# luoao-kddi/SCP

Hardware: AMD Instinct MI355X
Metric: KITTI frames/sec encode (SCP-EHEM, level 16) + bpp match vs ref (higher is better)
Workload: dtype f32 (dense layers and attention as bf16x3 split on bf16 MFMA, feature kNN as f16x3 split on f16 MFMA, fp32 accumulate; position kNN / CDF in fp32); 1 GPU; SCP-EHEM KITTI-like synthetic 120k-pt frames, --spher --mullevel lidar_level=16 (BASELINE.json configs[2]), seeded random weights; nodes_per_frame=577403, windows_per_frame=100, frames_per_gpu=46, frames_in_flight=4, frames_per_launch_sequence=1, transform=host-numpy on a prefetch thread (strict identity: the reference's integers), parallelism=frame-sharded x1, rank_cores=256, rank_cores_pinned=False

## Files before the change

### scp_amd/csrc/cdf.hip

```cpp
#include "scp_internal.h"

#define ROWS 64
#define MAXSYM 255

template <bool FROM_LOGITS>
__global__ __launch_bounds__(256) void cdf_kernel(const float *__restrict__ in, int64_t ld, int64_t n, int nsym,
                                                  const uint8_t *__restrict__ sym, float *__restrict__ pmf_out,
                                                  uint32_t *__restrict__ lohi, uint16_t *__restrict__ cdf_full) {
    __shared__ float tile[ROWS * MAXSYM];
    __shared__ float part[4 * ROWS];
    const int tid = threadIdx.x, lane = tid & 63, wq = tid >> 6;
    const int64_t row0 = (int64_t)blockIdx.x * ROWS;
    const int nrow = (int)((n - row0) < ROWS ? (n - row0) : ROWS);
    const int total = nrow * nsym;
    if (ld == nsym) {
        const float *src = in + row0 * ld;
        for (int i = tid; i < total; i += 256) tile[i] = src[i];
    } else if (ld == 256 && nsym <= 256 && (((uintptr_t)in) & 15) == 0) {
        for (int r = wq; r < nrow; r += 4) {
            const float4 v = *(const float4 *)(in + (row0 + r) * 256 + 4 * lane);
            const int c = 4 * lane;
            float *d = tile + r * nsym + c;
            if (c < nsym) d[0] = v.x;
            if (c + 1 < nsym) d[1] = v.y;
            if (c + 2 < nsym) d[2] = v.z;
            if (c + 3 < nsym) d[3] = v.w;
        }
    } else {
        for (int i = tid; i < total; i += 256) { const int r = i / nsym, c = i - r * nsym; tile[i] = in[(row0 + r) * ld + c]; }
    }
    __syncthreads();
    float *row = tile + lane * nsym;
// ... 41 lines not shown
            for (int u = 0; u < 8; ++u) v[u] = row[j + u];
#pragma unroll
            for (int u = 0; u < 8; ++u) { c = __fadd_rn(c, v[u]); v[u] = c; }
#pragma unroll
            for (int u = 0; u < 8; ++u) row[j + u] = v[u];
        }
        for (; j < nsym; ++j) { c = __fadd_rn(c, row[j]); row[j] = c; }
        const float c_last = c;
        const float c_lo = s > 0 ? row[s - 1] : 0.f, c_hi = row[s < nsym ? s : nsym - 1];
        if (lohi) {
            const double scale = (double)(65536 - nsym);
            const uint32_t lo = (s == 0) ? 0u : ((uint32_t)(int64_t)rint((double)(float)((double)c_lo / (double)c_last) * scale) + (uint32_t)s) & 0xFFFFu;
            uint32_t hi = ((uint32_t)(int64_t)rint((double)(float)((double)c_hi / (double)c_last) * scale) + (uint32_t)(s + 1)) & 0xFFFFu;
            if (s == nsym - 1) hi = 0u;
            lohi[row0 + lane] = lo | (hi << 16);
        }
    }
    if (cdf_full) {
        __syncthreads();
        const double scale = (double)(65536 - nsym);
        const int Lp = nsym + 1;
        for (int i = tid; i < nrow * Lp; i += 256) {
            const int r = i / Lp, k = i - r * Lp;
            uint32_t v = 0;
            if (k > 0) {
                const float last = tile[r * nsym + nsym - 1];
                v = ((uint32_t)(int64_t)rint((double)(float)((double)tile[r * nsym + k - 1] / (double)last) * scale) + (uint32_t)k) & 0xFFFFu;
            }
            cdf_full[(row0 + r) * Lp + k] = (uint16_t)v;
        }
    }
}

static int launch(bool from_logits, const float *in, int64_t ld, int64_t n, int32_t nsym, const uint8_t *sym, float *pmf,
                  uint32_t *lohi, uint16_t *cdf_full, void *stream) {
    if (n == 0) return SCP_OK;
    if (!in || n < 0 || nsym < 2 || nsym > MAXSYM || ld < nsym) return SCP_EINVAL;
    if (lohi && !sym) return SCP_EINVAL;
    const int nb = (int)cdiv64(n, ROWS);
    hipStream_t st = (hipStream_t)stream;
    SCP_PROF(SCP_PROF_CDF, st, (double)n * (4.0 * nsym + 4.0));
    if (from_logits) hipLaunchKernelGGL(cdf_kernel<true>, dim3(nb), dim3(256), 0, st, in, ld, n, nsym, sym, pmf, lohi, cdf_full);
    else hipLaunchKernelGGL(cdf_kernel<false>, dim3(nb), dim3(256), 0, st, in, ld, n, nsym, sym, pmf, lohi, cdf_full);
    LAUNCH_CHECK();
    return SCP_OK;
}

extern "C" int scp_softmax_cdf(const float *logits, int64_t ld, int64_t n, int32_t nsym, const uint8_t *sym, float *pmf,
                               uint32_t *lohi, uint16_t *cdf_full, void *stream) {
    return launch(true, logits, ld, n, nsym, sym, pmf, lohi, cdf_full, stream);
}

extern "C" int scp_pmf_cdf(const float *pmf, int64_t n, int32_t nsym, const uint8_t *sym, uint32_t *lohi, uint16_t *cdf_full,
                           void *stream) {
    return launch(false, pmf, nsym, n, nsym, sym, nullptr, lohi, cdf_full, stream);
}
```

### scp_amd/csrc/lnlin2.hip

```cpp
#include <stdlib.h>
#include <type_traits>
#include "rc_common.h"

#define L2_Q 16384
#define L2_OFF_BOUNCE (3 * L2_Q)
#define L2_OFF_BIAS (L2_OFF_BOUNCE + 4 * RC_BOUNCE)
#define L2_LDS (L2_OFF_BIAS + 8192)
static_assert(L2_LDS <= 80 * 1024, "two workgroups per CU: at most half of the 160 KiB");
#define L2_LDS_ONE (160 * 1024)

__device__ __forceinline__ void l2_issue(const RcLane &L, __amdgpu_buffer_rsrc_t wr_hi, __amdgpu_buffer_rsrc_t wr_lo, int j, int qt, char *dst) {
#pragma unroll
    for (int i = 0; i < 4; ++i) {
        const int b = i >> 1, plane = i & 1;
        const int soff = ((2 * j + b) * 16 + (L.w >> 1) * 8 + qt * 2 + (L.w & 1)) * 1024;
        __builtin_amdgcn_raw_ptr_buffer_load_lds(plane ? wr_lo : wr_hi, (rc_lds_ptr_t)(dst + (L.w + 4 * i) * 1024), 16, L.lane * 16, soff, 0, 0);
    }
}

#define L2_READ4(d0, d1, d2, d3, addr, o0, o1, o2, o3)                                                                                  \
    asm volatile("ds_read_b128 %0, %4 offset:%5\n\tds_read_b128 %1, %4 offset:%6\n\tds_read_b128 %2, %4 offset:%7\n\t"                      \
                 "ds_read_b128 %3, %4 offset:%8\n\ts_waitcnt lgkmcnt(0)"                                                                  \
                 : "=&v"(d0), "=&v"(d1), "=&v"(d2), "=&v"(d3) : "v"(addr), "n"(o0), "n"(o1), "n"(o2), "n"(o3) : "memory")
#define L2_READ4_AHEAD(d0, d1, d2, d3, addr, o0, o1, o2, o3)                                                                            \
    asm volatile("ds_read_b128 %0, %4 offset:%5\n\tds_read_b128 %1, %4 offset:%6\n\tds_read_b128 %2, %4 offset:%7\n\t"                      \
                 "ds_read_b128 %3, %4 offset:%8"                                                                                         \
                 : "=&v"(d0), "=&v"(d1), "=&v"(d2), "=&v"(d3) : "v"(addr), "n"(o0), "n"(o1), "n"(o2), "n"(o3) : "memory")
#define L2_WAIT4(d0, d1, d2, d3) asm volatile("s_waitcnt lgkmcnt(0)" : "+v"(d0), "+v"(d1), "+v"(d2), "+v"(d3) :: "memory")
#define L2_TOP(N) asm volatile("s_waitcnt vmcnt(" #N ") lgkmcnt(0)\n\ts_barrier" ::: "memory")

template <bool SWAP, int Q>
__device__ __forceinline__ void l2_quarter(unsigned ad0, unsigned ad1, rf32x16 &c0, rf32x16 &c1, const rbf16x8 (&Xh)[16], const rbf16x8 (&Xl)[16]) {
#define L2_MFMA(c, wf, xf) c = SWAP ? __builtin_amdgcn_mfma_f32_32x32x16_bf16(xf, wf, c, 0, 0, 0) : __builtin_amdgcn_mfma_f32_32x32x16_bf16(wf, xf, c, 0, 0, 0)
#define L2_FRAGS(M, A, ad, s) M(A[1], A[3], A[0], A[2], ad, 4096 + ((s) >> 1) * 1024, 12288 + ((s) >> 1) * 1024, ((s) >> 1) * 1024, 8192 + ((s) >> 1) * 1024)
    rbf16x8 A[2][4];
    L2_FRAGS(L2_READ4, A[0], ad0, 0);
#pragma unroll
    for (int s = 0; s < 4; ++s) {
        const int k = 4 * Q + s, n = (s + 1) & 1;
        if (s < 3) {
// ... 68 lines not shown
#pragma unroll
    for (int plane = 0; plane < 2; ++plane)
#pragma unroll
        for (int it = 0; it < 4; ++it)
            __builtin_amdgcn_raw_buffer_store_b128(y[plane][it], prs, L.lane * 16, it * 1024 + (vblk + head) * 4096 + (2 + plane) * pbytes, 0);
    asm volatile("s_waitcnt lgkmcnt(0)" ::: "memory");
}

template <bool KV>
__global__ __launch_bounds__(256, 2) void ln2_proj_kernel(const RcLnLinArgs a) {
    extern __shared__ __attribute__((aligned(1024))) char smem[];
    const RcLane L = rc_lane();
    const int ntiles = (a.M + RC_ROWS - 1) / RC_ROWS;
    const int nsteps = a.N >> 6;
    const int nq = KV ? a.nq : nsteps;
    char *bounce = smem + L2_OFF_BOUNCE + L.w * RC_BOUNCE;
    const unsigned ab = (unsigned)(uintptr_t)(rc_lds_ptr_t)smem + L.rg * 2048;
    const unsigned af0 = ab + L.frag, af1 = ab + (L.frag ^ 32);
    const unsigned asb = (unsigned)(uintptr_t)(rc_lds_ptr_t)(smem + L2_OFF_BIAS);
    const int ldo_bytes = (int)(a.ldo * 4);
    const int voff = (32 * L.w + (L.lane >> 3)) * ldo_bytes + (L.lane & 7) * 16;
    const int pbytes = (int)a.plane_bytes;
    const __amdgpu_buffer_rsrc_t prs = __builtin_amdgcn_make_buffer_rsrc((void *)a.planes, 0, (KV && !(a.probe & 1)) ? (int)(4 * a.plane_bytes) : 0, 0x00020000);
    const bool dma = !(a.probe & 2);

    const int wbytes = ((a.N + 255) & ~255) * 512;
    const __amdgpu_buffer_rsrc_t wr_hi = __builtin_amdgcn_make_buffer_rsrc((void *)a.Whi, 0, wbytes, 0x00020000);
    const __amdgpu_buffer_rsrc_t wr_lo = __builtin_amdgcn_make_buffer_rsrc((void *)a.Wlo, 0, wbytes, 0x00020000);

    float *sb = (float *)(smem + L2_OFF_BIAS), *sbw = sb + 1024;
    for (int i = threadIdx.x; i < a.N; i += 256) {
        const float b = a.bias ? a.bias[i] : 0.f;
        sb[i] = b; sbw[i] = b + (a.wbeta ? a.wbeta[i] : 0.f);
    }
    __syncthreads();
    int slot = 0;
    if (dma) { l2_issue(L, wr_hi, wr_lo, 0, 0, smem); l2_issue(L, wr_hi, wr_lo, 0, 1, smem + L2_Q); }
    for (int tile = blockIdx.x; tile < ntiles; tile += (int)gridDim.x) {
        const int m0 = tile * RC_ROWS;
        const int row = m0 + 32 * L.w + L.col;
        const int rowc = row < a.M ? row : a.M - 1;
        float keep = (row < a.M) ? 1.0f : 0.0f;
        if (a.valid) keep *= a.valid[rowc];
        rbf16x8 Xh[16], Xl[16];
        {
            float v[128];
            const float *src = a.x + (int64_t)((a.probe & 4) ? (rowc & 127) % a.M : rowc) * a.ldx + 8 * L.h;
#pragma unroll
            for (int s = 0; s < 16; ++s) {
                const rf32x4 q0 = *(const rf32x4 *)(src + 16 * s), q1 = *(const rf32x4 *)(src + 16 * s + 4);
#pragma unroll
                for (int u = 0; u < 4; ++u) { v[8 * s + u] = q0[u]; v[8 * s + 4 + u] = q1[u]; }
            }
            float mean, rstd;
            rc_ln_stats(v, a.eps, mean, rstd);
            const float sc = rstd * keep;
#pragma unroll
            for (int s = 0; s < 16; ++s) {
                float f[8];
#pragma unroll
                for (int i = 0; i < 8; ++i) f[i] = (v[8 * s + i] - mean) * sc;
                rc_split8(f, Xh[s], Xl[s]);
            }
        }
        const bool kept = keep != 0.f;
        const int64_t rows_left = (int64_t)a.M - m0;
        const int64_t span = (rows_left < RC_ROWS ? rows_left : RC_ROWS) * a.ldo * 4;
        const __amdgpu_buffer_rsrc_t rs = __builtin_amdgcn_make_buffer_rsrc(a.out + (int64_t)m0 * a.ldo, 0, (a.probe & 1) ? 0 : (int)span, 0x00020000);
        const unsigned kmask = (unsigned)__builtin_amdgcn_ballot_w64(kept);
        const unsigned maskh = kmask >> (4 * L.h);
        const int kvoff = (m0 + 32 * L.w + (L.lane >> 3)) * 512 + (L.lane & 7) * 16;
        const int vblk = ((m0 >> 5) + L.w) * 4;

        const unsigned atb = asb + (kept ? 4096 : 0) + 16 * L.h, atv = asb + 4 * L.col;
        rf32x16 c0, c1;
        auto bias_start = [&](int j) {
            if (KV && j >= nq + 4) {
                float bb[2], bwv[2];
                const unsigned ad = atv + 256 * j;
                asm volatile("ds_read_b32 %0, %4\n\tds_read_b32 %1, %4 offset:128\n\tds_read_b32 %2, %4 offset:4096\n\tds_read_b32 %3, %4 offset:4224\n\t"
                             "s_waitcnt lgkmcnt(0)" : "=&v"(bb[0]), "=&v"(bb[1]), "=&v"(bwv[0]), "=&v"(bwv[1]) : "v"(ad) : "memory");
#pragma unroll
                for (int blk = 0; blk < 2; ++blk) {
                    rf32x16 &c = blk ? c1 : c0;
#pragma unroll
                    for (int r = 0; r < 16; ++r) c[r] = ((maskh >> (8 * (r >> 2) + (r & 3))) & 1u) ? bwv[blk] : bb[blk];
                }
            } else {
                const unsigned ad = atb + 256 * j;
                rf32x4 t[2][4];
                L2_READ4(t[0][0], t[0][1], t[0][2], t[0][3], ad, 0, 32, 64, 96);
                L2_READ4(t[1][0], t[1][1], t[1][2], t[1][3], ad, 128, 160, 192, 224);
#pragma unroll
                for (int q = 0; q < 4; ++q)
#pragma unroll
                    for (int u = 0; u < 4; ++u) { c0[4 * q + u] = t[0][q][u]; c1[4 * q + u] = t[1][q][u]; }
            }
        };
        bias_start(0);
        SCP_WAIT_DMA(0);
        auto steps = [&](auto sw, int ja, int jb) {
// ... 16 lines not shown
            L2_QUARTER(3, 4)
#undef L2_QUARTER
            __builtin_amdgcn_sched_barrier(0);
            if (!SW && j < nq) {
#pragma unroll
                for (int blk = 0; blk < 2; ++blk) {
                    rf32x4 o[4];
#pragma unroll
                    for (int q = 0; q < 4; ++q)
#pragma unroll
                        for (int u = 0; u < 4; ++u) o[q][u] = (blk ? c1 : c0)[4 * q + u];
                    rc_store_block(L, bounce, o, rs, ldo_bytes, voff, 64 * j + 32 * blk);
                }
            } else if (!SW) {
                l2_store_k(L, bounce, c0, c1, prs, kvoff, pbytes, j - nq);
            } else {
                l2_store_v(L, bounce, c0, c1, prs, vblk, pbytes, j - nq - 4);
            }
            if (j + 1 < nsteps) bias_start(jn);
        }
        };
        if (KV) { steps(std::false_type(), 0, nq + 4); steps(std::true_type(), nq + 4, nsteps); }
        else steps(std::false_type(), 0, nsteps);
    }
    SCP_WAIT_DMA(0);
}

int scp_lnlin2_mode() {
    static int mode = -1;
    if (mode < 0) { const char *e = getenv("SCP_LNLIN"); mode = e ? atoi(e) : 0; if (mode < 0 || mode > 2) mode = 0; }
    return mode;
}

int scp_lnlin2_launch(RcLnLinArgs a, bool kv, int ncu, hipStream_t stream) {
    static int one = -1, probe = -1;
    if (one < 0) { const char *e = getenv("SCP_LNLIN_ONE"); one = (e && e[0] == '1') ? 1 : 0; }
    if (probe < 0) { const char *e = getenv("SCP_RC_PROBE"); probe = e ? atoi(e) : 0; }
    static bool configured = false;
    if (!configured) {
        HIP_TRY(hipFuncSetAttribute((const void *)ln2_proj_kernel<false>, hipFuncAttributeMaxDynamicSharedMemorySize, one ? L2_LDS_ONE : L2_LDS));
        HIP_TRY(hipFuncSetAttribute((const void *)ln2_proj_kernel<true>, hipFuncAttributeMaxDynamicSharedMemorySize, one ? L2_LDS_ONE : L2_LDS));
        configured = true;
    }
    a.ngroups = 1; a.probe = probe; a.dbg = nullptr;
    const int ntiles = (a.M + RC_ROWS - 1) / RC_ROWS;
    const int wgs = (one ? 1 : 2) * ncu;
    const dim3 grid((unsigned)(ntiles < wgs ? ntiles : wgs));
    if (kv) hipLaunchKernelGGL(ln2_proj_kernel<true>, grid, dim3(256), one ? L2_LDS_ONE : L2_LDS, stream, a);
    else hipLaunchKernelGGL(ln2_proj_kernel<false>, grid, dim3(256), one ? L2_LDS_ONE : L2_LDS, stream, a);
    LAUNCH_CHECK();
    return SCP_OK;
}
```

### scp_amd/csrc/rc_common.h

```cpp
#pragma once
#include "scp_internal.h"

typedef __bf16 rbf16x8 __attribute__((ext_vector_type(8)));
typedef float rf32x16 __attribute__((ext_vector_type(16)));
typedef float rf32x4 __attribute__((ext_vector_type(4)));
typedef int ri32x4 __attribute__((ext_vector_type(4)));
typedef __attribute__((address_space(3))) void *rc_lds_ptr_t;
typedef const __attribute__((address_space(1))) void *rc_glb_ptr_t;

#define RC_ROWS 128
#define RC_BOUNCE 4096

__device__ __forceinline__ void rc_dma16(const void *g, char *l) {
    __builtin_amdgcn_global_load_lds((rc_glb_ptr_t)g, (rc_lds_ptr_t)l, 16, 0, 0);
}

typedef float rf32x2 __attribute__((ext_vector_type(2)));
typedef __bf16 rbf16x2 __attribute__((ext_vector_type(2)));
typedef unsigned ru32x4 __attribute__((ext_vector_type(4)));
typedef unsigned ru32x2 __attribute__((ext_vector_type(2)));
__device__ __forceinline__ unsigned rc_pack2(float a, float b) {
    const rf32x2 v = {a, b};
    return __builtin_bit_cast(unsigned, __builtin_convertvector(v, rbf16x2));
}
// ... 38 lines not shown
        const int rho = 8 * it + (L.lane >> 3), kap = L.lane & 7;
        y[it] = *(const rf32x4 *)(bounce + rho * 128 + ((kap ^ (rho & 7)) << 4));
    }
#pragma unroll
    for (int it = 0; it < 4; ++it) __builtin_amdgcn_raw_buffer_store_b128(__builtin_bit_cast(ri32x4, y[it]), rs, voff, it * 8 * ldo_bytes + ch0 * 4, 0);
    asm volatile("s_waitcnt lgkmcnt(0)" ::: "memory");
}

__device__ __forceinline__ void rc_ln_stats(const float *v , float eps, float &mean, float &rstd) {
    float s = 0.f;
#pragma unroll
    for (int i = 0; i < 128; i += 4) s += (v[i] + v[i + 1]) + (v[i + 2] + v[i + 3]);
    s += __shfl_xor(s, 32);
    mean = s * (1.0f / 256.0f);
    float q = 0.f;
#pragma unroll
    for (int i = 0; i < 128; ++i) { const float d = v[i] - mean; q += d * d; }
    q += __shfl_xor(q, 32);
    rstd = rsqrtf(q * (1.0f / 256.0f) + eps);
}

struct RcLnLinArgs {
    const float *x; int64_t ldx;
    const float *valid;
    const __bf16 *Whi, *Wlo;
    const float *bias, *wbeta;
    float *out; int64_t ldo;
    int M, N;
    float eps;
    int probe;
    unsigned long long *dbg;
    __bf16 *planes; int64_t plane_bytes; int nq;
    int ngroups;
};

int scp_lnlin2_mode();
int scp_lnlin2_launch(RcLnLinArgs a, bool kv, int ncu, hipStream_t stream);
```

### scp_amd/csrc/rowchain.hip

```cpp
#include <stdlib.h>
#include "scp_internal.h"
#include "rc_common.h"

#define RC_SLOT 32768
#define RC_RING (4 * RC_SLOT)
#define RC_OFF_BOUNCE RC_RING
#define RC_OFF_BIAS (RC_RING + 4 * RC_BOUNCE)
#define RC_LDS (RC_OFF_BIAS + 16384)

__device__ __forceinline__ void rc_issue_rowchunk(const RcLane &L, const __bf16 *Whi, const __bf16 *Wlo, int g, char *slot) {
#pragma unroll
    for (int j = 0; j < 4; ++j) {
        const int p = L.w + 4 * j;
        const int64_t off = ((int64_t)g * 16 + p) * 512 + L.lane * 8;
        rc_dma16(Whi + off, slot + p * 1024);
        rc_dma16(Wlo + off, slot + 16384 + p * 1024);
    }
}

__device__ __forceinline__ void rc_issue_kchunk(const RcLane &L, const __bf16 *Whi, const __bf16 *Wlo, int c, int nks, char *slot) {
#pragma unroll
    for (int j = 0; j < 4; ++j) {
        const int p = L.w + 4 * j;
        const int64_t off = ((int64_t)p * nks + c) * 512 + L.lane * 8;
        rc_dma16(Whi + off, slot + p * 1024);
        rc_dma16(Wlo + off, slot + 16384 + p * 1024);
    }
}

__device__ __forceinline__ rbf16x8 rc_frag_rowchunk(const RcLane &L, const char *slot, int plane, int s) {
    return *(const rbf16x8 *)(slot + plane * 16384 + (L.rg * 8 + (s >> 1)) * 1024 + (L.frag ^ ((s & 1) << 5)));
}

__device__ __forceinline__ rbf16x8 rc_frag_kchunk(const RcLane &L, const char *slot, int plane, int b, int t) {
    return *(const rbf16x8 *)(slot + plane * 16384 + (2 * b + L.rg) * 1024 + (L.frag ^ (t << 5)));
}

#define RC_DS_READ4_WAIT(d0, a0, o0, d1, a1, o1, d2, a2, o2, d3, a3, o3)                                                              \
    asm volatile("ds_read_b128 %0, %4 offset:%8\n\tds_read_b128 %1, %5 offset:%9\n\tds_read_b128 %2, %6 offset:%10\n\t"                   \
                 "ds_read_b128 %3, %7 offset:%11\n\ts_waitcnt lgkmcnt(0)"                                                              \
                 : "=&v"(d0), "=&v"(d1), "=&v"(d2), "=&v"(d3) : "v"(a0), "v"(a1), "v"(a2), "v"(a3), "n"(o0), "n"(o1), "n"(o2), "n"(o3) : "memory")
// ... 133 lines not shown
                }
            }
            if (NSWAP && s == 14 && gap >= 4) {
                const float bb = sbn[32 * (gap - 4)], bwv = sbn[32 * (gap - 4) + 1024];
                rf32x16 &pp = (gap == 4) ? p0 : p1;
#pragma unroll
                for (int r = 0; r < 16; ++r) pp[r] = ((maskh >> (8 * (r >> 2) + (r & 3))) & 1u) ? bwv : bb;
            }
            if (!NSWAP && s == 14 && gap >= 4) {
#pragma unroll
                for (int q = 2 * (gap - 4); q < 2 * (gap - 4) + 2; ++q) {
                    const rf32x4 b0 = *(const rf32x4 *)(tb_next + 8 * q), b1 = *(const rf32x4 *)(tb_next + 32 + 8 * q);
#pragma unroll
                    for (int u = 0; u < 4; ++u) { p0[4 * q + u] = b0[u]; p1[4 * q + u] = b1[u]; }
                }
            }
            RC_SB;
        }
    }
    RC_DS_READ4_WAIT(A[0][1], an0, 16384, A[0][3], an0, RC_SLOT + 16384, A[0][0], an0, 0, A[0][2], an0, RC_SLOT);
    if (st) { const unsigned long long t = __builtin_amdgcn_s_memtime(); st[4] += t - ts0; }
}

template <int PROBE, bool KV = false>
__global__ __launch_bounds__(256, 1) void rc_ln_linear_kernel(const RcLnLinArgs a) {
    extern __shared__ __attribute__((aligned(1024))) char smem[];
    const RcLane L = rc_lane();
    const int ntiles = (a.M + RC_ROWS - 1) / RC_ROWS;
    const int nsteps = a.N >> 6;
    float *sb = (float *)(smem + RC_OFF_BIAS), *sbw = sb + 1024;
    for (int i = threadIdx.x; i < a.N; i += 256) {
        const float b = a.bias ? a.bias[i] : 0.f;
        sb[i] = b; sbw[i] = b + (a.wbeta ? a.wbeta[i] : 0.f);
    }
    __syncthreads();
    const int ngr = a.ngroups > 1 ? a.ngroups : 1;
    int tile = blockIdx.x / ngr;
    const int tstride = (int)gridDim.x / ngr;
    const int j0 = (int)(blockIdx.x % ngr) * (nsteps / ngr), j1 = j0 + nsteps / ngr;
    if (tile >= ntiles) return;
    char *bounce = smem + RC_OFF_BOUNCE + L.w * RC_BOUNCE;
    unsigned bw[4];
#pragma unroll
    for (int q = 0; q < 4; ++q) bw[q] = (unsigned)(uintptr_t)(rc_lds_ptr_t)(bounce + L.col * 128 + (((2 * q + L.h) ^ (L.col & 7)) << 4));
    const unsigned br0 = (unsigned)(uintptr_t)(rc_lds_ptr_t)(bounce + (L.lane >> 3) * 128 + (((L.lane & 7) ^ ((L.lane >> 3) & 7)) << 4));
    const int ldo_bytes = (int)(a.ldo * 4);
    const int voff = (32 * L.w + (L.lane >> 3)) * ldo_bytes + (L.lane & 7) * 16;
    const __amdgpu_buffer_rsrc_t rs_none = __builtin_amdgcn_make_buffer_rsrc(a.out, 0, 0, 0x00020000);
    const int pbytes = (int)a.plane_bytes;
    const __amdgpu_buffer_rsrc_t prs = __builtin_amdgcn_make_buffer_rsrc((void *)a.planes, 0, KV ? (int)(4 * a.plane_bytes) : 0, 0x00020000);

    const int wbytes = ((a.N + 255) & ~255) * 512;
    const __amdgpu_buffer_rsrc_t wr_hi = __builtin_amdgcn_make_buffer_rsrc((void *)a.Whi, 0, wbytes, 0x00020000);
    const __amdgpu_buffer_rsrc_t wr_lo = __builtin_amdgcn_make_buffer_rsrc((void *)a.Wlo, 0, wbytes, 0x00020000);
    unsigned long long t_step = 0, t_ln = 0, t_drain = 0, t_prev = 0, n_tiles = 0;
    unsigned long long tsl[5] = {0, 0, 0, 0, 0};
    const bool DBG = a.dbg != nullptr;
    if (DBG) t_prev = __builtin_amdgcn_s_memtime();
    auto stamp = [&](unsigned long long &acc_t) { if (DBG) { const unsigned long long t = __builtin_amdgcn_s_memtime(); acc_t += t - t_prev; t_prev = t; } };

    rc_issue_rowchunk(L, a.Whi, a.Wlo, 2 * j0, smem);
    rc_issue_rowchunk(L, a.Whi, a.Wlo, 2 * j0 + 1, smem + RC_SLOT);
    float v[128];
    auto xrow = [&](int t) {
        const int r = t * RC_ROWS + 32 * L.w + L.col;
        return a.x + (int64_t)(r < a.M ? r : a.M - 1) * a.ldx + 8 * L.h;
    };
    {
        const float *src = xrow(tile);
#pragma unroll
        for (int s = 0; s < 16; ++s) {
            const rf32x4 q0 = *(const rf32x4 *)(src + 16 * s), q1 = *(const rf32x4 *)(src + 16 * s + 4);
#pragma unroll
            for (int u = 0; u < 4; ++u) { v[8 * s + u] = q0[u]; v[8 * s + 4 + u] = q1[u]; }
        }
    }
    rbf16x8 A[2][4];
    {
        SCP_BARRIER_DMA(0);
        const unsigned ad0 = (unsigned)(uintptr_t)(rc_lds_ptr_t)(smem) + L.rg * 8192 + L.frag;
        RC_DS_READ4_WAIT(A[0][1], ad0, 16384, A[0][3], ad0, RC_SLOT + 16384, A[0][0], ad0, 0, A[0][2], ad0, RC_SLOT);
    }
    int gstep = 0;
    for (; tile < ntiles; tile += tstride) {
        const int m0 = tile * RC_ROWS;
        const int row = m0 + 32 * L.w + L.col;
        const int rowc = row < a.M ? row : a.M - 1;
        float keep = (row < a.M) ? 1.0f : 0.0f;
        if (a.valid) keep *= a.valid[rowc];
        float mean, rstd;
        rc_ln_stats(v, a.eps, mean, rstd);
        const float sc = rstd * keep;
        rbf16x8 Xh[16], Xl[16];
#pragma unroll
        for (int s = 0; s < 16; ++s) {
            float f[8];
#pragma unroll
            for (int i = 0; i < 8; ++i) f[i] = (v[8 * s + i] - mean) * sc;
            rc_split8(f, Xh[s], Xl[s]);
        }
        stamp(t_ln);
        const float *tb = (keep != 0.f ? sbw : sb) + 4 * L.h;
        const int64_t rows_left = (int64_t)a.M - m0;
        const int64_t span = (rows_left < RC_ROWS ? rows_left : RC_ROWS) * a.ldo * 4;
        const __amdgpu_buffer_rsrc_t rs = (a.probe & 1) ? rs_none : __builtin_amdgcn_make_buffer_rsrc(a.out + (int64_t)m0 * a.ldo, 0, (int)span, 0x00020000);
        const bool more = tile + tstride < ntiles;
        const float *xnext = xrow(more ? tile + tstride : tile);

        rf32x16 acc[2][2];
#pragma unroll
        for (int q = 0; q < 4; ++q) {
            const rf32x4 b0 = *(const rf32x4 *)(tb + 64 * j0 + 8 * q), b1 = *(const rf32x4 *)(tb + 64 * j0 + 32 + 8 * q);
#pragma unroll
            for (int u = 0; u < 4; ++u) { acc[0][0][4 * q + u] = b0[u]; acc[0][1][4 * q + u] = b1[u]; }
        }
        if (!KV) {
        for (int j = j0; j < j1; j += 2) {
            if (j + 2 == j1)
                rc_ll_step<true, PROBE>(L, a, smem, gstep & 1, acc[0][0], acc[0][1], acc[1][0], acc[1][1], Xh, Xl, 2 * (j + 1), j > j0 ? rs : rs_none, voff,
                                 ldo_bytes, 64 * (j - 1), bw, br0, xnext, v, A, tb + 64 * (j + 1), DBG ? tsl : nullptr, wr_hi, wr_lo);
            else
                rc_ll_step<false, PROBE>(L, a, smem, gstep & 1, acc[0][0], acc[0][1], acc[1][0], acc[1][1], Xh, Xl, 2 * (j + 1), j > j0 ? rs : rs_none, voff,
                                  ldo_bytes, 64 * (j - 1), bw, br0, xnext, v, A, tb + 64 * (j + 1), DBG ? tsl : nullptr, wr_hi, wr_lo);
            ++gstep;
            rc_ll_step<false, PROBE>(L, a, smem, gstep & 1, acc[1][0], acc[1][1], acc[0][0], acc[0][1], Xh, Xl, (j + 2 < j1) ? 2 * (j + 2) : 2 * j0, rs, voff,
                              ldo_bytes, 64 * j, bw, br0, xnext, v, A, tb + 64 * ((j + 2 < j1) ? j + 2 : j0), DBG ? tsl : nullptr, wr_hi, wr_lo);
            ++gstep;
        }
        stamp(t_step);
        asm volatile("s_waitcnt lgkmcnt(0)" ::: "memory");
#pragma unroll
        for (int blk = 0; blk < 2; ++blk) {
            rf32x4 o[4];
#pragma unroll
            for (int q = 0; q < 4; ++q)
#pragma unroll
                for (int u = 0; u < 4; ++u) o[q][u] = acc[1][blk][4 * q + u];
            rc_store_block(L, bounce, o, rs, ldo_bytes, voff, 64 * (j1 - 1) + 32 * blk);
        }
        } else {
// ... 79 lines not shown
                                                     br0, xnext, v, A, tbn, DBG ? tsl : nullptr, wr_hi, wr_lo, sbn2, maskh)
            if (!val) RC_STEP_A(false, false);
            else if (j + 2 == j1) RC_STEP_A(true, true);
            else RC_STEP_A(false, true);
            ++gstep;
            post(j, acc[0][0], acc[0][1]);
            if (!val) { if (nval) RC_STEP_B(false, true); else RC_STEP_B(false, false); }
            else { if (nval) RC_STEP_B(true, true); else RC_STEP_B(true, false); }
            ++gstep;
            post(j + 1, acc[1][0], acc[1][1]);
#undef RC_STEP_A
#undef RC_STEP_B
        }
        stamp(t_step);
        if (role(j1 - 1) == 0) {
            asm volatile("s_waitcnt lgkmcnt(0)" ::: "memory");
#pragma unroll
            for (int blk = 0; blk < 2; ++blk) {
                rf32x4 o[4];
#pragma unroll
                for (int q = 0; q < 4; ++q)
#pragma unroll
                    for (int u = 0; u < 4; ++u) o[q][u] = acc[1][blk][4 * q + u];
                rc_store_block(L, bounce, o, rs, ldo_bytes, voff, 64 * (j1 - 1) + 32 * blk);
            }
        }
        }
        stamp(t_drain);
        ++n_tiles;
    }
    if (DBG && L.lane == 0) {
        unsigned long long *o = a.dbg + ((size_t)blockIdx.x * 4 + L.w) * 8;
        o[0] = tsl[3]; o[1] = t_step; o[2] = t_ln; o[3] = t_drain; o[4] = n_tiles; o[5] = tsl[0]; o[6] = tsl[1]; o[7] = tsl[2] + tsl[4];
    }
    SCP_WAIT_DMA(0);
}

struct RcPostArgs {
    const __bf16 *Ohi, *Olo; int64_t ldo_in;
    const float *x; int64_t ldx;
    const void *W;
    const float *bp, *b1, *b2;
    float *out; int64_t ldc;
    int M;
    float eps;
    unsigned long long *dbg;
    int dbg_mode;
    const int32_t *tile_list; int n_list;
};

#define RC_W_PROJ 0
#define RC_W_FC1 (256 * 512)
#define RC_W_FC2 (RC_W_FC1 + 1024 * 512)
#define RC_W_PLANE (RC_W_FC2 + 256 * 2048)
struct RcSlotSrc { int base, stride; };

__device__ __forceinline__ void rc_dma_piece(const RcLane &L, __amdgpu_buffer_rsrc_t wr, const RcSlotSrc &src, char *slot_lds, int s, int plane) {
    const int pb = L.w + 4 * (s & 3);
    const int soff = src.base + pb * src.stride + plane * RC_W_PLANE;
    __builtin_amdgcn_raw_ptr_buffer_load_lds(wr, (rc_lds_ptr_t)(slot_lds + plane * 16384 + pb * 1024), 16, L.lane * 16, soff, 0, 0);
}

struct RcFragAddr { unsigned r0, r1, k0, k1; };
__device__ __forceinline__ RcFragAddr rc_frag_addr(const RcLane &L, char *half_base) {
    RcFragAddr f;
    const unsigned b = (unsigned)(uintptr_t)(rc_lds_ptr_t)half_base;
// ... 1007 lines not shown
    if (g_rc_wide == -2) { const char *e = getenv("SCP_RC_WIDE"); g_rc_wide = e ? atoi(e) : -1; if (g_rc_wide < -1 || g_rc_wide > 1) g_rc_wide = -1; }
    return g_rc_wide;
}
extern "C" SCP_API int scp_rc_set_wide(int32_t mode) { g_rc_wide = (mode < -1 || mode > 1) ? -1 : mode; return SCP_OK; }
extern "C" SCP_API int scp_rc_set_grid(int32_t workgroups) { g_rc_grid = workgroups > 0 ? workgroups : 0; return SCP_OK; }
static int rc_num_cu() {
    if (g_rc_grid) return g_rc_grid;
    if (!g_rc_num_cu) {
        int dev = 0;
        hipDeviceProp_t p;
        if (hipGetDevice(&dev) != hipSuccess || hipGetDeviceProperties(&p, dev) != hipSuccess) return 256;
        g_rc_num_cu = p.multiProcessorCount > 0 ? p.multiProcessorCount : 256;
    }
    return g_rc_num_cu;
}

static bool rc_lnlin2_here(int ntiles, int ncu) {
    const int mode = scp_lnlin2_mode();
    return mode == 2 || (mode == 0 && 4 * (int64_t)ntiles >= 3 * (int64_t)ncu);
}

extern "C" SCP_API int scp_swin_ln_linear(const float *x, int64_t ldx, const float *valid, const void *Whi, const void *Wlo, const float *bias,
                                          const float *wbeta, float eps, float *out, int64_t ldo, int32_t M, int32_t N, void *stream) {
    if (!x || !Whi || !Wlo || !out || M <= 0 || N <= 0 || (N & 127) || N > 1024 || ldx < 256 || (ldx & 3) || ldo < N || (ldo & 3) ||
        (((uintptr_t)x | (uintptr_t)out | (uintptr_t)Whi | (uintptr_t)Wlo) & 15) || (int64_t)RC_ROWS * ldo * 4 > 0x7fffffffLL)
        return SCP_EINVAL;
    static bool configured = false;
    if (!configured) {
        HIP_TRY(hipFuncSetAttribute((const void *)rc_ln_linear_kernel<0>, hipFuncAttributeMaxDynamicSharedMemorySize, RC_LDS));
        configured = true;
    }
    RcLnLinArgs a;
    a.x = x; a.ldx = ldx; a.valid = valid; a.Whi = (const __bf16 *)Whi; a.Wlo = (const __bf16 *)Wlo; a.bias = bias; a.wbeta = wbeta;
    a.out = out; a.ldo = ldo; a.M = M; a.N = N; a.eps = eps;
    a.planes = nullptr; a.plane_bytes = 0; a.nq = 0;
    { static int pr = -1; if (pr < 0) { const char *e = getenv("SCP_RC_PROBE"); pr = e ? atoi(e) : 0; } a.probe = pr; }
    if (a.probe) { const char *e = getenv("SCP_RC_PROBE"); a.probe = e ? atoi(e) : 0; }
    a.dbg = g_rc_dbg;
    const int ntiles = (M + RC_ROWS - 1) / RC_ROWS;
    const int ncu = rc_num_cu();
    SCP_PROF(SCP_PROF_LN_LINEAR, stream, 2.0 * M * 256.0 * N);
    if (rc_lnlin2_here(ntiles, ncu)) return scp_lnlin2_launch(a, false, ncu, (hipStream_t)stream);
    a.ngroups = rc_ll_groups(ntiles, N / 64, ncu);
    hipLaunchKernelGGL(rc_ln_linear_kernel<0>, dim3((unsigned)(a.ngroups > 1 ? ntiles * a.ngroups : (ntiles < ncu ? ntiles : ncu))), dim3(256), RC_LDS, (hipStream_t)stream, a);
    LAUNCH_CHECK();
    return SCP_OK;
}

extern "C" SCP_API int scp_swin_ln_qkv(const float *x, int64_t ldx, const float *valid, const void *Whi, const void *Wlo, const float *bias,
                                       const float *wbeta, float eps, float *q, int64_t ldq, void *planes, int64_t Tp, int32_t M, int32_t N, void *stream) {
    if (!x || !Whi || !Wlo || !planes || M <= 0 || (M & 127) || (N != 768 && N != 512) || (N == 768 && (!q || ldq < 256 || (ldq & 3))) || ldx < 256 ||
        (ldx & 3) || Tp < M || (Tp & 31) || (((uintptr_t)x | (uintptr_t)q | (uintptr_t)Whi | (uintptr_t)Wlo | (uintptr_t)planes) & 15) ||
        (q && (int64_t)RC_ROWS * ldq * 4 > 0x7fffffffLL) || 4 * Tp * 512 > 0x7fffffffLL)
        return SCP_EINVAL;
    static bool configured = false;
    if (!configured) {
        HIP_TRY(hipFuncSetAttribute((const void *)rc_ln_linear_kernel<0, true>, hipFuncAttributeMaxDynamicSharedMemorySize, RC_LDS));
        configured = true;
    }
    RcLnLinArgs a;
    a.x = x; a.ldx = ldx; a.valid = valid; a.Whi = (const __bf16 *)Whi; a.Wlo = (const __bf16 *)Wlo; a.bias = bias; a.wbeta = wbeta;
    a.out = q; a.ldo = q ? ldq : 256; a.M = M; a.N = N; a.eps = eps; a.probe = 0; a.dbg = nullptr;
    a.planes = (__bf16 *)planes; a.plane_bytes = Tp * 512; a.nq = N / 64 - 8;
    const int ntiles = M / RC_ROWS, ncu = rc_num_cu();
    SCP_PROF(SCP_PROF_LN_LINEAR, stream, 2.0 * M * 256.0 * N);
    if (rc_lnlin2_here(ntiles, ncu)) return scp_lnlin2_launch(a, true, ncu, (hipStream_t)stream);
    a.ngroups = rc_ll_groups(ntiles, N / 64, ncu);
    hipLaunchKernelGGL((rc_ln_linear_kernel<0, true>), dim3((unsigned)(a.ngroups > 1 ? ntiles * a.ngroups : (ntiles < ncu ? ntiles : ncu))), dim3(256), RC_LDS, (hipStream_t)stream, a);
    LAUNCH_CHECK();
    return SCP_OK;
}

extern "C" SCP_API int scp_swin_post_attn(const void *Ohi, const void *Olo, int64_t ldo_in, const float *x, int64_t ldx, const void *W, const float *bp,
                                          const float *b1, const float *b2, float eps, float *out, int64_t ldc, int32_t M, const int32_t *tile_list,
                                          int32_t n_tiles, void *stream) {
    if (!Ohi || !Olo || !x || !W || !bp || !b1 || !b2 || !out || M <= 0 || (tile_list && (n_tiles <= 0 || n_tiles > (M + RC_ROWS - 1) / RC_ROWS)) || ldo_in < 256 || (ldo_in & 7) || ldx < 256 || (ldx & 3) || ldc < 256 ||
        (ldc & 3) || (((uintptr_t)Ohi | (uintptr_t)Olo | (uintptr_t)x | (uintptr_t)out | (uintptr_t)W) & 15) ||
        (int64_t)RC_ROWS * ldc * 4 > 0x7fffffffLL)
        return SCP_EINVAL;
    static bool configured = false;
    if (!configured) {
        HIP_TRY(hipFuncSetAttribute((const void *)rc_post_attn_kernel, hipFuncAttributeMaxDynamicSharedMemorySize, RC_LDS));
        HIP_TRY(hipFuncSetAttribute((const void *)rc_post_attn_wide_kernel, hipFuncAttributeMaxDynamicSharedMemorySize, RC_LDS));
        configured = true;
    }
    RcPostArgs a;
    a.Ohi = (const __bf16 *)Ohi; a.Olo = (const __bf16 *)Olo; a.ldo_in = ldo_in; a.x = x; a.ldx = ldx; a.W = W;
    a.bp = bp; a.b1 = b1; a.b2 = b2; a.out = out; a.ldc = ldc; a.M = M; a.eps = eps;
    a.dbg = g_rc_dbg;
    { const char *e = getenv("SCP_RC_DUMP"); a.dbg_mode = e ? atoi(e) : 0; }
    a.tile_list = tile_list; a.n_list = tile_list ? n_tiles : 0;
    const int ntiles = tile_list ? n_tiles : (M + RC_ROWS - 1) / RC_ROWS;
    const int ncu = rc_num_cu();
    SCP_PROF(SCP_PROF_POST_ATTN, stream, 2.0 * (tile_list ? (double)n_tiles * RC_ROWS : (double)M) * (256.0 * 256.0 + 2.0 * 256.0 * 1024.0));
    if (rc_wide_mode() == 1 || (rc_wide_mode() < 0 && !g_rc_dbg && !a.dbg_mode && 4 * (int64_t)ntiles <= (int64_t)ncu)) {
// ... 69 lines not shown
```

Baseline: 15.31 frames/s.

## Skip GEMM on all-padding row tiles and add register-resident softmax-CDF kernel

In the LN+linear row-chain and lnlin2 kernels, tiles whose rows are all invalid (padding) skip the LayerNorm and MFMA work. Their outputs are written straight from the bias, including pre-split bf16 hi/lo K/V plane values. Separately, the softmax-to-lohi CDF path gets a one-wave-per-64-rows kernel that transposes logits through a small LDS buffer into per-thread registers and computes max, exp, sum and the cumulative lo/hi without a 255-float LDS tile per row. Both are meant to cut wasted compute and LDS traffic, but they add register pressure (256 floats per thread) and depend on padding-row outputs exactly matching what the full computation would produce.

```diff
diff --git a/scp_amd/csrc/cdf.hip b/scp_amd/csrc/cdf.hip
--- a/scp_amd/csrc/cdf.hip
+++ b/scp_amd/csrc/cdf.hip
@@ -1,3 +1,4 @@
+#include <stdlib.h>
 #include "scp_internal.h"
 
 #define ROWS 64
@@ -105,6 +106,80 @@
     }
 }
 
+#define LH_CH 32
+#define LH_LD (LH_CH + 1)
+template <bool FULL>
+__global__ __launch_bounds__(64) void cdf_lohi_kernel(const float *__restrict__ in, int64_t n, int nsym, const uint8_t *__restrict__ sym,
+                                                     uint32_t *__restrict__ lohi) {
+    __shared__ float tr[64 * LH_LD];
+    const int lane = threadIdx.x;
+    const int64_t row0 = (int64_t)blockIdx.x * 64;
+    float x[256];
+    {
+        const float *src[8];
+#pragma unroll
+        for (int it = 0; it < 8; ++it) {
+            int64_t r = row0 + 8 * it + (lane >> 3);
+            r = r < n ? r : n - 1;
+            src[it] = in + r * 256 + 4 * (lane & 7);
+        }
+        float4 t[2][8];
+#pragma unroll
+        for (int it = 0; it < 8; ++it) t[0][it] = *(const float4 *)(src[it]);
+#pragma unroll
+        for (int k = 0; k < 256 / LH_CH; ++k) {
+            if (k + 1 < 256 / LH_CH) {
+#pragma unroll
+                for (int it = 0; it < 8; ++it) t[(k + 1) & 1][it] = *(const float4 *)(src[it] + LH_CH * (k + 1));
+            }
+            if (k) __syncthreads();
+#pragma unroll
+            for (int it = 0; it < 8; ++it) {
+                float *d = tr + (8 * it + (lane >> 3)) * LH_LD + 4 * (lane & 7);
+                const float4 v = t[k & 1][it];
+                d[0] = v.x; d[1] = v.y; d[2] = v.z; d[3] = v.w;
+            }
+            __syncthreads();
+#pragma unroll
+            for (int c = 0; c < LH_CH; ++c) x[LH_CH * k + c] = tr[lane * LH_LD + c];
+        }
+    }
+#pragma unroll
+    for (int j = 0; j < 256; ++j)
+        if (FULL ? j >= 255 : j >= nsym) x[j] = -INFINITY;
+    float m = -INFINITY;
+#pragma unroll
+    for (int j = 0; j < 256; ++j) m = fmaxf(m, x[j]);
+    float sum = 0.f;
+#pragma unroll
+    for (int j = 0; j < 256; ++j) { x[j] = expf(x[j] - m); sum = __fadd_rn(sum, x[j]); }
+    if (row0 + lane >= n) return;
+    const int s = (int)sym[row0 + lane];
+    float c = 0.f, c_lo = 0.f, c_hi = 0.f;
+    int sk = s;
+#pragma unroll
+    for (int j = 0; j < 256; ++j) {
+        if ((j & 7) == 0) asm volatile("" : "+v"(sk), "+v"(c_lo), "+v"(c_hi) : "v"(c));
+        const float prev = c;
+        c = __fadd_rn(c, x[j] / sum);
+        const bool here = (j == sk);
+        c_lo = here ? prev : c_lo;
+        c_hi = here ? c : c_hi;
+    }
+    const float c_last = c;
+    const double scale = (double)(65536 - nsym);
+    const uint32_t lo = (s == 0) ? 0u : ((uint32_t)(int64_t)rint((double)(float)((double)c_lo / (double)c_last) * scale) + (uint32_t)s) & 0xFFFFu;
+    uint32_t hi = ((uint32_t)(int64_t)rint((double)(float)((double)c_hi / (double)c_last) * scale) + (uint32_t)(s + 1)) & 0xFFFFu;
+    if (s == nsym - 1) hi = 0u;
+    lohi[row0 + lane] = lo | (hi << 16);
+}
+
+static bool cdf_lohi_on() {
+    static int on = -1;
+    if (on < 0) { const char *e = getenv("SCP_CDF"); on = (e && e[0] == 'o') ? 0 : 1; }
+    return on != 0;
+}
+
 static int launch(bool from_logits, const float *in, int64_t ld, int64_t n, int32_t nsym, const uint8_t *sym, float *pmf,
                   uint32_t *lohi, uint16_t *cdf_full, void *stream) {
     if (n == 0) return SCP_OK;
@@ -113,6 +188,12 @@
     const int nb = (int)cdiv64(n, ROWS);
     hipStream_t st = (hipStream_t)stream;
     SCP_PROF(SCP_PROF_CDF, st, (double)n * (4.0 * nsym + 4.0));
+    if (from_logits && lohi && !pmf && !cdf_full && ld == 256 && (((uintptr_t)in) & 15) == 0 && cdf_lohi_on()) {
+        if (nsym == 255) hipLaunchKernelGGL(cdf_lohi_kernel<true>, dim3(nb), dim3(64), 0, st, in, n, nsym, sym, lohi);
+        else hipLaunchKernelGGL(cdf_lohi_kernel<false>, dim3(nb), dim3(64), 0, st, in, n, nsym, sym, lohi);
+        LAUNCH_CHECK();
+        return SCP_OK;
+    }
     if (from_logits) hipLaunchKernelGGL(cdf_kernel<true>, dim3(nb), dim3(256), 0, st, in, ld, n, nsym, sym, pmf, lohi, cdf_full);
     else hipLaunchKernelGGL(cdf_kernel<false>, dim3(nb), dim3(256), 0, st, in, ld, n, nsym, sym, pmf, lohi, cdf_full);
     LAUNCH_CHECK();
diff --git a/scp_amd/csrc/lnlin2.hip b/scp_amd/csrc/lnlin2.hip
--- a/scp_amd/csrc/lnlin2.hip
+++ b/scp_amd/csrc/lnlin2.hip
@@ -5,7 +5,8 @@
 #define L2_Q 16384
 #define L2_OFF_BOUNCE (3 * L2_Q)
 #define L2_OFF_BIAS (L2_OFF_BOUNCE + 4 * RC_BOUNCE)
-#define L2_LDS (L2_OFF_BIAS + 8192)
+#define L2_OFF_PAD (L2_OFF_BIAS + 8192)
+#define L2_LDS (L2_OFF_PAD + 2048)
 static_assert(L2_LDS <= 80 * 1024, "two workgroups per CU: at most half of the 160 KiB");
 #define L2_LDS_ONE (160 * 1024)
 
@@ -140,12 +141,20 @@
     for (int i = threadIdx.x; i < a.N; i += 256) {
         const float b = a.bias ? a.bias[i] : 0.f;
         sb[i] = b; sbw[i] = b + (a.wbeta ? a.wbeta[i] : 0.f);
+        if (KV) rc_pad_fill(smem + L2_OFF_PAD, i, nq, b);
     }
     __syncthreads();
     int slot = 0;
     if (dma) { l2_issue(L, wr_hi, wr_lo, 0, 0, smem); l2_issue(L, wr_hi, wr_lo, 0, 1, smem + L2_Q); }
     for (int tile = blockIdx.x; tile < ntiles; tile += (int)gridDim.x) {
         const int m0 = tile * RC_ROWS;
+        const int64_t rows_left = (int64_t)a.M - m0;
+        const int64_t span = (rows_left < RC_ROWS ? rows_left : RC_ROWS) * a.ldo * 4;
+        const __amdgpu_buffer_rsrc_t rs = __builtin_amdgcn_make_buffer_rsrc(a.out + (int64_t)m0 * a.ldo, 0, (a.probe & 1) ? 0 : (int)span, 0x00020000);
+        if (rc_tile_allpad(a, m0, L.lane)) {
+            rc_pad_tile(L, sb, smem + L2_OFF_PAD, m0, 0, nsteps, nq, rs, ldo_bytes, voff, prs, pbytes);
+            continue;
+        }
         const int row = m0 + 32 * L.w + L.col;
         const int rowc = row < a.M ? row : a.M - 1;
         float keep = (row < a.M) ? 1.0f : 0.0f;
@@ -172,9 +181,6 @@
             }
         }
         const bool kept = keep != 0.f;
-        const int64_t rows_left = (int64_t)a.M - m0;
-        const int64_t span = (rows_left < RC_ROWS ? rows_left : RC_ROWS) * a.ldo * 4;
-        const __amdgpu_buffer_rsrc_t rs = __builtin_amdgcn_make_buffer_rsrc(a.out + (int64_t)m0 * a.ldo, 0, (a.probe & 1) ? 0 : (int)span, 0x00020000);
         const unsigned kmask = (unsigned)__builtin_amdgcn_ballot_w64(kept);
         const unsigned maskh = kmask >> (4 * L.h);
         const int kvoff = (m0 + 32 * L.w + (L.lane >> 3)) * 512 + (L.lane & 7) * 16;
@@ -257,6 +263,12 @@
     return mode;
 }
 
+int scp_padskip() {
+    static int on = -1;
+    if (on < 0) { const char *e = getenv("SCP_PADSKIP"); on = (e && e[0] == '0') ? 0 : 1; }
+    return on;
+}
+
 int scp_lnlin2_launch(RcLnLinArgs a, bool kv, int ncu, hipStream_t stream) {
     static int one = -1, probe = -1;
     if (one < 0) { const char *e = getenv("SCP_LNLIN_ONE"); one = (e && e[0] == '1') ? 1 : 0; }
@@ -267,7 +279,7 @@
         HIP_TRY(hipFuncSetAttribute((const void *)ln2_proj_kernel<true>, hipFuncAttributeMaxDynamicSharedMemorySize, one ? L2_LDS_ONE : L2_LDS));
         configured = true;
     }
-    a.ngroups = 1; a.probe = probe; a.dbg = nullptr;
+    a.ngroups = 1; a.probe = probe; a.dbg = nullptr; a.padskip = scp_padskip();
     const int ntiles = (a.M + RC_ROWS - 1) / RC_ROWS;
     const int wgs = (one ? 1 : 2) * ncu;
     const dim3 grid((unsigned)(ntiles < wgs ? ntiles : wgs));
diff --git a/scp_amd/csrc/rc_common.h b/scp_amd/csrc/rc_common.h
--- a/scp_amd/csrc/rc_common.h
+++ b/scp_amd/csrc/rc_common.h
@@ -94,7 +94,64 @@
     unsigned long long *dbg;
     __bf16 *planes; int64_t plane_bytes; int nq;
     int ngroups;
+    int padskip;
 };
+
+__device__ __forceinline__ bool rc_tile_allpad(const RcLnLinArgs &a, int m0, int lane) {
+    if (!a.padskip || !a.valid) return false;
+    const int r0 = m0 + lane, r1 = r0 + 64;
+    const bool k0 = r0 < a.M && a.valid[r0] != 0.f, k1 = r1 < a.M && a.valid[r1] != 0.f;
+    return __builtin_amdgcn_ballot_w64(k0 || k1) == 0;
+}
+
+__device__ __forceinline__ void rc_pad_fill(char *pad, int i, int nq, float b) {
+    const int c = i - 64 * nq;
+    if (c < 0) return;
+    const float b0 = b + 0.0f;
+    const unsigned hi = rc_pack2(b0, 0.f) & 0xffffu, lo = rc_pack2(b0 - __builtin_bit_cast(float, hi << 16), 0.f) & 0xffffu;
+    unsigned short *t = (unsigned short *)pad + (c >> 8) * 512 + (c & 255);
+    t[0] = (unsigned short)hi; t[256] = (unsigned short)lo;
+}
+
+__device__ __forceinline__ void rc_pad_tile(const RcLane &L, const float *sb, const char *pad, int m0, int ja, int jb, int nq, __amdgpu_buffer_rsrc_t rs,
+                                            int ldo_bytes, int voff, __amdgpu_buffer_rsrc_t prs, int pbytes) {
+    const int sw = (L.lane & 7) ^ ((L.lane >> 3) & 7);
+    for (int j = ja; j < jb; ++j) {
+        if (j < nq) {
+#pragma unroll
+            for (int blk = 0; blk < 2; ++blk) {
+                const int ch0 = 64 * j + 32 * blk;
+                rf32x4 y = *(const rf32x4 *)(sb + ch0 + 4 * (L.lane & 7));
+#pragma unroll
+                for (int u = 0; u < 4; ++u) y[u] += 0.0f;
+#pragma unroll
+                for (int it = 0; it < 4; ++it) __builtin_amdgcn_raw_buffer_store_b128(__builtin_bit_cast(ri32x4, y), rs, voff, it * 8 * ldo_bytes + ch0 * 4, 0);
+            }
+        } else if (j < nq + 4) {
+            const int head = j - nq;
+            const int kvoff = (m0 + 32 * L.w + (L.lane >> 3)) * 512 + (L.lane & 7) * 16;
+#pragma unroll
+            for (int plane = 0; plane < 2; ++plane) {
+                const ri32x4 y = *(const ri32x4 *)(pad + plane * 512 + head * 128 + 16 * sw);
+#pragma unroll
+                for (int it = 0; it < 4; ++it) __builtin_amdgcn_raw_buffer_store_b128(y, prs, kvoff, it * 8 * 512 + head * 128 + plane * pbytes, 0);
+            }
+        } else {
+            const int head = j - nq - 4;
+            const int vblk = ((m0 >> 5) + L.w) * 4;
+#pragma unroll
+            for (int plane = 0; plane < 2; ++plane)
+#pragma unroll
+                for (int it = 0; it < 4; ++it) {
+                    const int d = 2 * (8 * it + (L.lane >> 3)) + (sw >> 2);
+                    const int w2 = (int)(*(const unsigned short *)(pad + (2 + plane) * 512 + (head * 64 + d) * 2)) * 0x10001;
+                    __builtin_amdgcn_raw_buffer_store_b128((ri32x4){w2, w2, w2, w2}, prs, L.lane * 16, it * 1024 + (vblk + head) * 4096 + (2 + plane) * pbytes, 0);
+                }
+        }
+    }
+}
+
+int scp_padskip();
 
 int scp_lnlin2_mode();
 int scp_lnlin2_launch(RcLnLinArgs a, bool kv, int ncu, hipStream_t stream);
diff --git a/scp_amd/csrc/rowchain.hip b/scp_amd/csrc/rowchain.hip
--- a/scp_amd/csrc/rowchain.hip
+++ b/scp_amd/csrc/rowchain.hip
@@ -7,6 +7,7 @@
 #define RC_OFF_BOUNCE RC_RING
 #define RC_OFF_BIAS (RC_RING + 4 * RC_BOUNCE)
 #define RC_LDS (RC_OFF_BIAS + 16384)
+#define RC_OFF_PAD (RC_OFF_BIAS + 8192)
 
 __device__ __forceinline__ void rc_issue_rowchunk(const RcLane &L, const __bf16 *Whi, const __bf16 *Wlo, int g, char *slot) {
 #pragma unroll
@@ -206,23 +207,37 @@
     for (int i = threadIdx.x; i < a.N; i += 256) {
         const float b = a.bias ? a.bias[i] : 0.f;
         sb[i] = b; sbw[i] = b + (a.wbeta ? a.wbeta[i] : 0.f);
+        if (KV) rc_pad_fill(smem + RC_OFF_PAD, i, a.nq, b);
     }
     __syncthreads();
     const int ngr = a.ngroups > 1 ? a.ngroups : 1;
     int tile = blockIdx.x / ngr;
     const int tstride = (int)gridDim.x / ngr;
     const int j0 = (int)(blockIdx.x % ngr) * (nsteps / ngr), j1 = j0 + nsteps / ngr;
-    if (tile >= ntiles) return;
-    char *bounce = smem + RC_OFF_BOUNCE + L.w * RC_BOUNCE;
-    unsigned bw[4];
-#pragma unroll
-    for (int q = 0; q < 4; ++q) bw[q] = (unsigned)(uintptr_t)(rc_lds_ptr_t)(bounce + L.col * 128 + (((2 * q + L.h) ^ (L.col & 7)) << 4));
-    const unsigned br0 = (unsigned)(uintptr_t)(rc_lds_ptr_t)(bounce + (L.lane >> 3) * 128 + (((L.lane & 7) ^ ((L.lane >> 3) & 7)) << 4));
     const int ldo_bytes = (int)(a.ldo * 4);
     const int voff = (32 * L.w + (L.lane >> 3)) * ldo_bytes + (L.lane & 7) * 16;
     const __amdgpu_buffer_rsrc_t rs_none = __builtin_amdgcn_make_buffer_rsrc(a.out, 0, 0, 0x00020000);
     const int pbytes = (int)a.plane_bytes;
     const __amdgpu_buffer_rsrc_t prs = __builtin_amdgcn_make_buffer_rsrc((void *)a.planes, 0, KV ? (int)(4 * a.plane_bytes) : 0, 0x00020000);
+    auto out_rows = [&](int t) {
+        const int64_t rows_left = (int64_t)a.M - (int64_t)t * RC_ROWS;
+        const int64_t span = (rows_left < RC_ROWS ? rows_left : RC_ROWS) * a.ldo * 4;
+        return (a.probe & 1) ? rs_none : __builtin_amdgcn_make_buffer_rsrc(a.out + (int64_t)t * RC_ROWS * a.ldo, 0, (int)span, 0x00020000);
+    };
+    auto next_real = [&](int t) {
+        while (t < ntiles && rc_tile_allpad(a, t * RC_ROWS, L.lane)) {
+            rc_pad_tile(L, sb, smem + RC_OFF_PAD, t * RC_ROWS, j0, j1, KV ? a.nq : nsteps, out_rows(t), ldo_bytes, voff, prs, pbytes);
+            t += tstride;
+        }
+        return t;
+    };
+    tile = next_real(tile);
+    if (tile < ntiles) {
+    char *bounce = smem + RC_OFF_BOUNCE + L.w * RC_BOUNCE;
+    unsigned bw[4];
+#pragma unroll
+    for (int q = 0; q < 4; ++q) bw[q] = (unsigned)(uintptr_t)(rc_lds_ptr_t)(bounce + L.col * 128 + (((2 * q + L.h) ^ (L.col & 7)) << 4));
+    const unsigned br0 = (unsigned)(uintptr_t)(rc_lds_ptr_t)(bounce + (L.lane >> 3) * 128 + (((L.lane & 7) ^ ((L.lane >> 3) & 7)) << 4));
 
     const int wbytes = ((a.N + 255) & ~255) * 512;
     const __amdgpu_buffer_rsrc_t wr_hi = __builtin_amdgcn_make_buffer_rsrc((void *)a.Whi, 0, wbytes, 0x00020000);
@@ -256,7 +271,7 @@
         RC_DS_READ4_WAIT(A[0][1], ad0, 16384, A[0][3], ad0, RC_SLOT + 16384, A[0][0], ad0, 0, A[0][2], ad0, RC_SLOT);
     }
     int gstep = 0;
-    for (; tile < ntiles; tile += tstride) {
+    for (int tnext; tile < ntiles; tile = tnext) {
         const int m0 = tile * RC_ROWS;
         const int row = m0 + 32 * L.w + L.col;
         const int rowc = row < a.M ? row : a.M - 1;
@@ -275,11 +290,10 @@
         }
         stamp(t_ln);
         const float *tb = (keep != 0.f ? sbw : sb) + 4 * L.h;
-        const int64_t rows_left = (int64_t)a.M - m0;
-        const int64_t span = (rows_left < RC_ROWS ? rows_left : RC_ROWS) * a.ldo * 4;
-        const __amdgpu_buffer_rsrc_t rs = (a.probe & 1) ? rs_none : __builtin_amdgcn_make_buffer_rsrc(a.out + (int64_t)m0 * a.ldo, 0, (int)span, 0x00020000);
-        const bool more = tile + tstride < ntiles;
-        const float *xnext = xrow(more ? tile + tstride : tile);
+        const __amdgpu_buffer_rsrc_t rs = out_rows(tile);
+        tnext = next_real(tile + tstride);
+        const bool more = tnext < ntiles;
+        const float *xnext = xrow(more ? tnext : tile);
 
         rf32x16 acc[2][2];
 #pragma unroll
@@ -425,6 +439,7 @@
     if (DBG && L.lane == 0) {
         unsigned long long *o = a.dbg + ((size_t)blockIdx.x * 4 + L.w) * 8;
         o[0] = tsl[3]; o[1] = t_step; o[2] = t_ln; o[3] = t_drain; o[4] = n_tiles; o[5] = tsl[0]; o[6] = tsl[1]; o[7] = tsl[2] + tsl[4];
+    }
     }
     SCP_WAIT_DMA(0);
 }
@@ -1498,7 +1513,7 @@
     }
     RcLnLinArgs a;
     a.x = x; a.ldx = ldx; a.valid = valid; a.Whi = (const __bf16 *)Whi; a.Wlo = (const __bf16 *)Wlo; a.bias = bias; a.wbeta = wbeta;
-    a.out = out; a.ldo = ldo; a.M = M; a.N = N; a.eps = eps;
+    a.out = out; a.ldo = ldo; a.M = M; a.N = N; a.eps = eps; a.padskip = scp_padskip();
     a.planes = nullptr; a.plane_bytes = 0; a.nq = 0;
     { static int pr = -1; if (pr < 0) { const char *e = getenv("SCP_RC_PROBE"); pr = e ? atoi(e) : 0; } a.probe = pr; }
     if (a.probe) { const char *e = getenv("SCP_RC_PROBE"); a.probe = e ? atoi(e) : 0; }
@@ -1526,7 +1541,7 @@
     }
     RcLnLinArgs a;
     a.x = x; a.ldx = ldx; a.valid = valid; a.Whi = (const __bf16 *)Whi; a.Wlo = (const __bf16 *)Wlo; a.bias = bias; a.wbeta = wbeta;
-    a.out = q; a.ldo = q ? ldq : 256; a.M = M; a.N = N; a.eps = eps; a.probe = 0; a.dbg = nullptr;
+    a.out = q; a.ldo = q ? ldq : 256; a.M = M; a.N = N; a.eps = eps; a.probe = 0; a.dbg = nullptr; a.padskip = scp_padskip();
     a.planes = (__bf16 *)planes; a.plane_bytes = Tp * 512; a.nq = N / 64 - 8;
     const int ntiles = M / RC_ROWS, ncu = rc_num_cu();
     SCP_PROF(SCP_PROF_LN_LINEAR, stream, 2.0 * M * 256.0 * N);
```

After: 15.33 frames/s, median of 4. No clear change (+0.1%).
